# cmhungsteve/TA3N

Measured on NVIDIA H100. Metric: video-clips/sec fwd+bwd (B=256,T=5,D=2048), higher is better.
Workload: dtype tf32x3

## Files before the change

### include/ta3n_b200.h

```cpp
#ifndef TA3N_B200_H_
#define TA3N_B200_H_

#include <stddef.h>
#include <stdint.h>

#ifdef __cplusplus
extern "C" {
#endif

#define TA3N_ABI_VERSION 3

enum {
  TA3N_OK = 0,
  TA3N_ERR_INVALID = 1,
  TA3N_ERR_WORKSPACE = 2,
  TA3N_ERR_CUDA = 3,
  TA3N_ERR_UNSUPPORTED = 4
};

enum {
  TA3N_GEMM_FP32_SIMT = 0,
  TA3N_GEMM_TF32_TCGEN05 = 1,
  TA3N_GEMM_TF32X3_TCGEN05 = 2
};

typedef void* ta3n_stream_t;

typedef struct {
  int num_frames;
  int n_scales;
  const int* scale_size;
  const int* rel_count;
  const int* frames;
} ta3n_relation_table;

typedef struct {
  float p;
  const uint8_t* keep;
  uint64_t seed;
  const uint64_t* step_dev;
} ta3n_dropout;

int ta3n_abi_version(void);
const char* ta3n_last_error(void);
uint64_t ta3n_launch_count(void);
void ta3n_reset_launch_count(void);
int ta3n_set_gemm_engine(int engine);
int ta3n_get_gemm_engine(void);
int ta3n_set_forward_scratch(void* scratch, size_t bytes);
int ta3n_plan_forward_splits(int n_groups, const int* M, const int* N, const int* K, int sms, size_t scratch_bytes,
                             int* ksplit_out, double* makespan_out);
void ta3n_timing_enable(int on);
size_t ta3n_timing_report(char* buf, size_t buf_bytes);

int ta3n_shared_fc_fwd(const float* x_src, int rows_src, const float* x_tgt, int rows_tgt, int D,
                       const float* W, const float* b, int F, const ta3n_dropout* drop,
                       float* feat, ta3n_stream_t stream);
size_t ta3n_shared_fc_bwd_workspace_bytes(int rows, int D, int F);
int ta3n_shared_fc_bwd(const float* x_src, int rows_src, const float* x_tgt, int rows_tgt, int D,
                       int F, const float* feat, float* dfeat, const float* g_feat_ext, float p,
                       float* dW, float* db, void* workspace, size_t workspace_bytes,
                       ta3n_stream_t stream);

int ta3n_disc_fwd(const float* x, int rows, int K, int Kh, const float* W1, const float* b1,
                  const float* W2, const float* b2, float* hidden, float* logits,
                  ta3n_stream_t stream);
size_t ta3n_disc_bwd_workspace_bytes(int rows, int K, int Kh);
int ta3n_disc_bwd(const float* x, int rows, int K, int Kh, const float* W1, const float* W2,
                  const float* hidden, const float* g_logits, float beta, float* dx,
                  int accumulate, float* dW1, float* db1, float* dW2, float* db2,
                  void* workspace, size_t workspace_bytes, ta3n_stream_t stream);
int ta3n_grl_bwd(const float* g, float beta, float* out, size_t n, ta3n_stream_t stream);

int ta3n_frame_attn_fwd(const float* feat, const float* logits, int rows, int F, float* out,
                        ta3n_stream_t stream);
int ta3n_frame_attn_bwd(const float* feat, const float* logits, int rows, int F, float* d_out,
                        float* g_logits, ta3n_stream_t stream);

int ta3n_segment_mean_fwd(const float* x, int M, int T, int F, float* out, ta3n_stream_t stream);
int ta3n_segment_mean_bwd(const float* g, int M, int T, int F, float* dx, ta3n_stream_t stream);

int ta3n_trn_fwd(const float* x, int M, int F, int H, const ta3n_relation_table* tab,
                 const float* const* W_host, const float* const* b_host, int relu_input,
                 float* act, float* feat_rel, ta3n_stream_t stream);
size_t ta3n_trn_bwd_workspace_bytes(int M, int F, int H, const ta3n_relation_table* tab);
int ta3n_trn_bwd(const float* x, int M, int F, int H, const ta3n_relation_table* tab,
                 const float* const* W_host, int relu_input, const float* act,
                 const float* d_feat_rel, float* const* dW_host, float* const* db_host, float* dx,
                 int accumulate_dx, void* workspace, size_t workspace_bytes, ta3n_stream_t stream);

int ta3n_relattn_fwd(const float* feat_rel, int M, int R, int H, const float* const* W1_host,
                     const float* const* b1_host, const float* const* W2_host,
                     const float* const* b2_host, int use_attn, float* hidden, float* pred_rel,
                     float* attn, float* feat_video, ta3n_stream_t stream);
size_t ta3n_relattn_bwd_workspace_bytes(int M, int R, int H);
int ta3n_relattn_bwd(const float* feat_rel, int M, int R, int H, const float* const* W1_host,
                     const float* const* W2_host, int use_attn, const float* hidden,
                     const float* pred_rel, const float* attn, const float* g_feat_video,
                     const float* g_pred_rel, const float* g_attn, float beta,
                     float* d_feat_rel, float* const* dW1_host, float* const* db1_host,
                     float* const* dW2_host, float* const* db2_host, void* workspace,
                     size_t workspace_bytes, ta3n_stream_t stream);

int ta3n_general_attn_fwd(const float* feat_rel, int M, int R, int H, const float* W1, const float* b1,
                          const float* w2, const float* b2, float* hidden, float* attn, float* feat_video,
                          ta3n_stream_t stream);
size_t ta3n_general_attn_bwd_workspace_bytes(int M, int R, int H);
int ta3n_general_attn_bwd(const float* feat_rel, int M, int R, int H, const float* W1, const float* w2,
                          const float* hidden, const float* attn, const float* g_feat_video, const float* g_attn,
                          float* d_feat_rel, float* dW1, float* db1, float* dw2, float* db2, void* workspace,
                          size_t workspace_bytes, ta3n_stream_t stream);

int ta3n_video_head_fwd(const float* feat_video, int M, int H, int C, const float* Wc,
                        const float* bc, const ta3n_dropout* drop, float* dropped, float* pred,
                        ta3n_stream_t stream);
size_t ta3n_video_head_bwd_workspace_bytes(int M, int H, int C);
int ta3n_video_head_bwd(const float* dropped, int M, int H, int C, const float* Wc,
                        const ta3n_dropout* drop, const float* g_pred,
                        const float* d_dropped_extra, const float* g_feat_video_ext,
                        float grad_scale, float* d_feat_video, float* dWc, float* dbc,
                        void* workspace, size_t workspace_bytes, ta3n_stream_t stream);

int ta3n_fwd_batch_begin(void);
size_t ta3n_fwd_batch_workspace_bytes(void);
int ta3n_fwd_batch_flush(void* workspace, size_t workspace_bytes, ta3n_stream_t stream);

int ta3n_wgrad_defer_begin(void);
size_t ta3n_wgrad_defer_workspace_bytes(void);
int ta3n_wgrad_defer_flush(void* workspace, size_t workspace_bytes, ta3n_stream_t stream);

size_t ta3n_loss_workspace_bytes(int M);
int ta3n_loss_fwd_bwd(const float* pred_video, const long long* labels, const float* pred_rel,
                      const float* pred_dom_video, const float* pred_frame, int Bs, int Bt, int T,
                      int R, int C, float gamma, int flags, const int* valid_rows, float* loss,
                      float* g_pred_video,
                      float* g_pred_rel, float* g_pred_dom_video, float* g_pred_frame,
                      void* workspace, size_t workspace_bytes, ta3n_stream_t stream);
int ta3n_counter_inc(uint64_t* counter, ta3n_stream_t stream);

typedef struct {
  int Bs, Bt;
  int T, D, F, H, C;
  int use_attn;
  int loss_flags;
  float gamma;
  float domain_weight[2];
  const float* class_weight;
  const float* beta_dev;
  const ta3n_relation_table* tab;
  const float* x_src;
  const float* x_tgt;
  const long long* labels;
  const int* valid_rows;
  ta3n_dropout drop_i, drop_v;
  const float *W_sh, *b_sh;
  const float *W1f, *b1f, *W2f, *b2f;
  const float* const* W_trn_host;
  const float* const* b_trn_host;
  const float* const* W1r_host;
  const float* const* b1r_host;
  const float* const* W2r_host;
  const float* const* b2r_host;
  const float *Wc, *bc;
  const float *W1v, *b1v, *W2v, *b2v;
  float *dW_sh, *db_sh, *dW1f, *db1f, *dW2f, *db2f;
  float* const* dW_trn_host;
  float* const* db_trn_host;
  float* const* dW1r_host;
  float* const* db1r_host;
  float* const* dW2r_host;
  float* const* db2r_host;
  float *dWc, *dbc, *dW1v, *db1v, *dW2v, *db2v;
  float* feat;
  float* hid_f;
  float* pred_frame;
  float* act;
  float* feat_rel;
  float* hid_r;
  float* pred_rel;
  float* attn;
  float* feat_video;
  float* dropped;
  float* pred_video;
  float* hid_v;
  float* pred_dom;
  float* loss;
  uint64_t* step_counter;
  void* workspace;
  size_t workspace_bytes;
} ta3n_step_desc;

size_t ta3n_step_workspace_bytes(const ta3n_step_desc* desc);
int ta3n_step_run_phased(const ta3n_step_desc* desc, ta3n_stream_t stream);

size_t ta3n_allreduce_flag_bytes(int world);
int ta3n_allreduce_mean(float* const* peer_bufs_host, float* multicast_buf, uint32_t* const* peer_flags_host,
                        const uint64_t* seq_dev, int rank, int world, long long n, ta3n_stream_t stream);

size_t ta3n_sgd_workspace_bytes(void);
// ... 20 lines not shown
```

### ta3n_b200/_lib.py

```python
from __future__ import annotations

import ctypes as C
import os
import threading

from . import build as _build

ABI_VERSION = 3

TA3N_GEMM_FP32_SIMT = 0
TA3N_GEMM_TF32_TCGEN05 = 1
TA3N_GEMM_TF32X3_TCGEN05 = 2


class RelationTable(C.Structure):
    _fields_ = [("num_frames", C.c_int), ("n_scales", C.c_int),
                ("scale_size", C.POINTER(C.c_int)), ("rel_count", C.POINTER(C.c_int)),
                ("frames", C.POINTER(C.c_int))]


class Dropout(C.Structure):
    _fields_ = [("p", C.c_float), ("keep", C.c_void_p), ("seed", C.c_uint64), ("step_dev", C.c_void_p)]


class StepDesc(C.Structure):
    _fields_ = (
        [(n, C.c_int) for n in ("Bs", "Bt", "T", "D", "F", "H", "C", "use_attn", "loss_flags")] +
        [("gamma", C.c_float), ("domain_weight", C.c_float * 2), ("class_weight", C.c_void_p),
         ("beta_dev", C.c_void_p), ("tab", C.POINTER(RelationTable)),
         ("x_src", C.c_void_p), ("x_tgt", C.c_void_p), ("labels", C.c_void_p), ("valid_rows", C.c_void_p),
         ("drop_i", Dropout), ("drop_v", Dropout)] +
        [(n, C.c_void_p) for n in ("W_sh", "b_sh", "W1f", "b1f", "W2f", "b2f")] +
        [(n, C.POINTER(C.c_void_p)) for n in ("W_trn_host", "b_trn_host", "W1r_host", "b1r_host", "W2r_host",
                                              "b2r_host")] +
        [(n, C.c_void_p) for n in ("Wc", "bc", "W1v", "b1v", "W2v", "b2v")] +
        [(n, C.c_void_p) for n in ("dW_sh", "db_sh", "dW1f", "db1f", "dW2f", "db2f")] +
        [(n, C.POINTER(C.c_void_p)) for n in ("dW_trn_host", "db_trn_host", "dW1r_host", "db1r_host", "dW2r_host",
                                              "db2r_host")] +
        [(n, C.c_void_p) for n in ("dWc", "dbc", "dW1v", "db1v", "dW2v", "db2v")] +
        [(n, C.c_void_p) for n in ("feat", "hid_f", "pred_frame", "act", "feat_rel", "hid_r", "pred_rel", "attn",
                                   "feat_video", "dropped", "pred_video", "hid_v", "pred_dom", "loss",
                                   "step_counter", "workspace")] +
        [("workspace_bytes", C.c_size_t)])


_VP, _I, _F, _SZ = C.c_void_p, C.c_int, C.c_float, C.c_size_t
_IP = C.POINTER(C.c_int)
_PP = C.POINTER(C.c_void_p)
_TAB = C.POINTER(RelationTable)
_DRP = C.POINTER(Dropout)

SIGNATURES = {
    "ta3n_abi_version": (_I, []),
    "ta3n_last_error": (C.c_char_p, []),
    "ta3n_launch_count": (C.c_uint64, []),
    "ta3n_reset_launch_count": (None, []),
    "ta3n_set_gemm_engine": (_I, [_I]),
    "ta3n_get_gemm_engine": (_I, []),
    "ta3n_set_forward_scratch": (_I, [_VP, _SZ]),
    "ta3n_plan_forward_splits": (_I, [_I, _IP, _IP, _IP, _I, _SZ, _IP, C.POINTER(C.c_double)]),
    "ta3n_timing_enable": (None, [_I]),
    "ta3n_timing_report": (_SZ, [C.c_char_p, _SZ]),
    "ta3n_shared_fc_fwd": (_I, [_VP, _I, _VP, _I, _I, _VP, _VP, _I, _DRP, _VP, _VP]),
    "ta3n_shared_fc_bwd_workspace_bytes": (_SZ, [_I, _I, _I]),
    "ta3n_shared_fc_bwd": (_I, [_VP, _I, _VP, _I, _I, _I, _VP, _VP, _VP, _F, _VP, _VP, _VP, _SZ, _VP]),
    "ta3n_disc_fwd": (_I, [_VP, _I, _I, _I, _VP, _VP, _VP, _VP, _VP, _VP, _VP]),
    "ta3n_disc_bwd_workspace_bytes": (_SZ, [_I, _I, _I]),
    "ta3n_disc_bwd": (_I, [_VP, _I, _I, _I, _VP, _VP, _VP, _VP, _F, _VP, _I, _VP, _VP, _VP, _VP, _VP, _SZ, _VP]),
    "ta3n_grl_bwd": (_I, [_VP, _F, _VP, _SZ, _VP]),
    "ta3n_frame_attn_fwd": (_I, [_VP, _VP, _I, _I, _VP, _VP]),
    "ta3n_frame_attn_bwd": (_I, [_VP, _VP, _I, _I, _VP, _VP, _VP]),
    "ta3n_segment_mean_fwd": (_I, [_VP, _I, _I, _I, _VP, _VP]),
    "ta3n_segment_mean_bwd": (_I, [_VP, _I, _I, _I, _VP, _VP]),
    "ta3n_trn_fwd": (_I, [_VP, _I, _I, _I, _TAB, _PP, _PP, _I, _VP, _VP, _VP]),
    "ta3n_trn_bwd_workspace_bytes": (_SZ, [_I, _I, _I, _TAB]),
    "ta3n_trn_bwd": (_I, [_VP, _I, _I, _I, _TAB, _PP, _I, _VP, _VP, _PP, _PP, _VP, _I, _VP, _SZ, _VP]),
    "ta3n_relattn_fwd": (_I, [_VP, _I, _I, _I, _PP, _PP, _PP, _PP, _I, _VP, _VP, _VP, _VP, _VP]),
    "ta3n_relattn_bwd_workspace_bytes": (_SZ, [_I, _I, _I]),
    "ta3n_relattn_bwd": (_I, [_VP, _I, _I, _I, _PP, _PP, _I, _VP, _VP, _VP, _VP, _VP, _VP, _F, _VP,
                              _PP, _PP, _PP, _PP, _VP, _SZ, _VP]),
    "ta3n_general_attn_fwd": (_I, [_VP, _I, _I, _I, _VP, _VP, _VP, _VP, _VP, _VP, _VP, _VP]),
    "ta3n_general_attn_bwd_workspace_bytes": (_SZ, [_I, _I, _I]),
    "ta3n_general_attn_bwd": (_I, [_VP, _I, _I, _I, _VP, _VP, _VP, _VP, _VP, _VP, _VP, _VP, _VP, _VP, _VP, _VP, _SZ, _VP]),
    "ta3n_video_head_fwd": (_I, [_VP, _I, _I, _I, _VP, _VP, _DRP, _VP, _VP, _VP]),
    "ta3n_video_head_bwd_workspace_bytes": (_SZ, [_I, _I, _I]),
    "ta3n_video_head_bwd": (_I, [_VP, _I, _I, _I, _VP, _DRP, _VP, _VP, _VP, _F, _VP, _VP, _VP, _VP, _SZ, _VP]),
    "ta3n_fwd_batch_begin": (_I, []),
    "ta3n_fwd_batch_workspace_bytes": (_SZ, []),
    "ta3n_fwd_batch_flush": (_I, [_VP, _SZ, _VP]),
    "ta3n_wgrad_defer_begin": (_I, []),
    "ta3n_wgrad_defer_workspace_bytes": (_SZ, []),
    "ta3n_wgrad_defer_flush": (_I, [_VP, _SZ, _VP]),
    "ta3n_loss_workspace_bytes": (_SZ, [_I]),
    "ta3n_loss_fwd_bwd": (_I, [_VP, _VP, _VP, _VP, _VP, _I, _I, _I, _I, _I, _F, _I, _VP, _VP, _VP, _VP, _VP, _VP,
                               _VP, _SZ, _VP]),
    "ta3n_counter_inc": (_I, [_VP, _VP]),
    "ta3n_step_workspace_bytes": (_SZ, [C.POINTER(StepDesc)]),
    "ta3n_step_run_phased": (_I, [C.POINTER(StepDesc), _VP]),
    "ta3n_allreduce_flag_bytes": (_SZ, [_I]),
    "ta3n_allreduce_mean": (_I, [_PP, _VP, _PP, _VP, _I, _I, C.c_longlong, _VP]),
    "ta3n_sgd_workspace_bytes": (_SZ, []),
    "ta3n_sgd_nesterov_step": (_I, [_VP, _VP, _VP, C.c_longlong, _VP, _F, _F, _F, _VP, _SZ, _VP, _VP]),
    "ta3n_sgd_nesterov_step_masked": (_I, [_VP, _VP, _VP, C.c_longlong, _VP, _F, _F, _F, _VP, _SZ, _VP, _VP, _VP]),
    "ta3n_gemm_tn": (_I, [_VP, _VP, _VP, _I, _I, _I, _VP]),
    "ta3n_gemm_ex": (_I, [_VP, _I, _I, _VP, _I, _I, _VP, _I, _I, _I, _I, _VP, _SZ, _VP]),
}

_lock = threading.Lock()
_lib = None


class Ta3nError(RuntimeError):
    pass


def lib_path() -> str:
    return os.environ.get("TA3N_LIB", _build.LIB_PATH)


def load() -> C.CDLL:
    global _lib
    if _lib is not None:
        return _lib
    with _lock:
        if _lib is None:
            path = lib_path()
            if not os.path.exists(path):
                raise Ta3nError(
                    f"{path} is missing: build it with `python -m ta3n_b200.build` "
                    "(or __graft_entry__.build()). ta3n_b200 has no CPU / PyTorch fallback.")
            lib = C.CDLL(path)
            for name, (res, args) in SIGNATURES.items():
                fn = getattr(lib, name)
                fn.restype = res
                fn.argtypes = args
            if lib.ta3n_abi_version() != ABI_VERSION:
                raise Ta3nError("libta3n_sm90.so ABI version mismatch")
            _lib = lib
    return _lib


def check(rc: int) -> None:
    if rc != 0:
        msg = load().ta3n_last_error()
        raise Ta3nError(f"libta3n_sm90 error {rc}: {msg.decode() if msg else '?'}")


def ptr_array(ptrs):
    arr = (C.c_void_p * len(ptrs))(*ptrs)
    return arr


def set_gemm_engine(engine) -> None:
    code = {"fp32": TA3N_GEMM_FP32_SIMT, "tf32": TA3N_GEMM_TF32_TCGEN05, "tf32x3": TA3N_GEMM_TF32X3_TCGEN05}.get(engine, engine)
    check(load().ta3n_set_gemm_engine(int(code)))


def get_gemm_engine() -> str:
    return {0: "fp32", 1: "tf32", 2: "tf32x3"}[load().ta3n_get_gemm_engine()]


def plan_forward_splits(shapes, sms: int = 132, scratch_bytes: int = 48 << 20):
    n = len(shapes)
    arr = lambda col: (C.c_int * n)(*[int(s[col]) for s in shapes])
    ks, span = (C.c_int * n)(), (C.c_double * 2)()
    check(load().ta3n_plan_forward_splits(n, arr(0), arr(1), arr(2), int(sms), int(scratch_bytes), ks, span))
    return list(ks), span[0], span[1]

# ... 22 lines not shown
```

### ta3n_b200/build.py

```python
from __future__ import annotations

import os
import shutil
import subprocess
import sys

PKG_DIR = os.path.dirname(os.path.abspath(__file__))
CSRC = os.path.join(PKG_DIR, "csrc")
LIB_PATH = os.path.join(PKG_DIR, "libta3n_sm90.so")
SOURCES = ["ta3n_api.cu"]
HEADERS = ["common.cuh", "seg_gemm.cuh", "rowops.cuh", "gemm_wgmma.cuh", "optim.cuh", "step_rows.cuh",
           "step_plan.cuh", "allreduce.cuh",
           os.path.join("..", "..", "include", "ta3n_b200.h")]
NVCC_FLAGS = [
    "-gencode", "arch=compute_90a,code=sm_90a", "-lineinfo", "-O3", "-std=c++17",
    "-Xcompiler", "-fPIC", "-shared",
]


def _nvcc() -> str:
    for cand in (shutil.which("nvcc"), "/usr/local/cuda/bin/nvcc"):
        if cand and os.path.exists(cand):
            return cand
    raise RuntimeError("nvcc not found; cannot build libta3n_sm90.so")


def needs_build() -> bool:
    if not os.path.exists(LIB_PATH):
        return True
    t = os.path.getmtime(LIB_PATH)
    deps = [os.path.join(CSRC, s) for s in SOURCES + HEADERS]
    return any(os.path.getmtime(d) > t for d in deps if os.path.exists(d))


def build(force: bool = False, verbose: bool = False) -> str:
    if not force and not needs_build():
        return LIB_PATH
    cmd = [_nvcc(), *NVCC_FLAGS, *[os.path.join(CSRC, s) for s in SOURCES], "-o", LIB_PATH]
    if verbose:
        cmd.insert(1, "-Xptxas")
        cmd.insert(2, "-v")
        print(" ".join(cmd), file=sys.stderr)
    res = subprocess.run(cmd, capture_output=True, text=True)
    if res.returncode != 0:
        raise RuntimeError("nvcc failed:\n" + res.stdout + res.stderr)
    if verbose:
        print(res.stderr, file=sys.stderr)
    return LIB_PATH


if __name__ == "__main__":
    print(build(force="--force" in sys.argv, verbose=True))
```

### ta3n_b200/csrc/ta3n_api.cu

```cuda
#include "common.cuh"
#include "seg_gemm.cuh"
#include "rowops.cuh"
#include "gemm_wgmma.cuh"
#include "optim.cuh"
#include "step_plan.cuh"
#include "allreduce.cuh"

#include <functional>

using namespace ta3n;

namespace {

struct RelLayout {
  int T, R, n_rel, n_slots;
  std::vector<int> scale_size, rel_count, rel_begin;
  std::vector<int> rel_scale;
  std::vector<int> slot_begin;
  const int* frames;
};

int parse_table(const ta3n_relation_table* tab, RelLayout* L) {
  TA3N_REQUIRE(tab != nullptr, "relation table is null");
  TA3N_REQUIRE(tab->num_frames >= 2 && tab->n_scales >= 1 && tab->n_scales <= kMaxScales, "bad table sizes");
  TA3N_REQUIRE(tab->scale_size && tab->rel_count && tab->frames, "relation table arrays are null");
  L->T = tab->num_frames;
  L->R = tab->n_scales;
  L->frames = tab->frames;
  L->n_rel = 0;
  L->n_slots = 0;
  for (int i = 0; i < L->R; ++i) {
    const int s = tab->scale_size[i], n = tab->rel_count[i];
    TA3N_REQUIRE(s >= 1 && s <= L->T && n >= 1, "bad scale entry");
    L->scale_size.push_back(s);
    L->rel_count.push_back(n);
    L->rel_begin.push_back(L->n_rel);
    for (int r = 0; r < n; ++r) {
      L->rel_scale.push_back(i);
      L->slot_begin.push_back(L->n_slots);
      for (int j = 0; j < s; ++j) {
        const int t = tab->frames[L->n_slots + j];
        TA3N_REQUIRE(t >= 0 && t < L->T, "frame id out of range");
      }
      L->n_slots += s;
    }
    L->n_rel += n;
  }
  L->rel_begin.push_back(L->n_rel);
  TA3N_REQUIRE(L->n_rel <= kMaxRel, "too many relations");
  return TA3N_OK;
}

RelMap make_relmap(const RelLayout& L) {
  RelMap m;
  memset(&m, 0, sizeof(m));
  m.n_rel = L.n_rel;
  m.n_scales = L.R;
  for (int i = 0; i <= L.R; ++i) m.rel_begin[i] = L.rel_begin[i];
  for (int q = 0; q < L.n_rel; ++q) m.scale_of[q] = (unsigned char)L.rel_scale[q];
  return m;
}

void set_dropout_epilogue(Group& g, const DropArgs& d, const uint8_t* keep, int ldkeep, uint64_t rng_offset) {
  if (d.mode == 0) return;
  g.drop_scale = d.scale;
  g.drop_p = d.p;
  if (d.mode == 1) {
    g.flags |= EPI_DROP_MASK;
    g.keep = keep;
    g.ldkeep = ldkeep;
  } else {
    g.flags |= EPI_DROP_RNG;
    g.seed = d.seed;
    g.step_dev = d.step_dev;
    g.rng_offset = rng_offset;
  }
}

inline cudaStream_t S(ta3n_stream_t s) { return static_cast<cudaStream_t>(s); }

inline size_t splitk_bytes(int n_groups) {
  return (size_t)2 * 296 * 128 * 128 * sizeof(float) + (size_t)256 * (n_groups + 1) + 4096;
}

struct DeferCtx {
// ... 644 lines not shown
    plan.precise = true;
    Group& g = plan.add_group(M * R, H, hidden, H);
    g.flags = EPI_BIAS;
    g.bias = b1;
    plan.add_seg(feat_rel, H, W1, H, H);
    TA3N_TRY(run_gemm(plan, S(stream)));
  }
  pre_launch("general_attn_rows", S(stream));
  launch_kernel(general_attn_fwd_kernel, M, 32 * (R < kRelWarps ? R : kRelWarps), 0, S(stream), feat_rel, hidden, M, R,
                H, w2, b2, attn, feat_video);
  return after_launch();
}

size_t ta3n_general_attn_bwd_workspace_bytes(int M, int R, int H) {
  return Arena::round((size_t)M * R * H * sizeof(float)) + Arena::round((size_t)M * R * sizeof(float)) +
         splitk_bytes(1) + colsum_bytes((size_t)2 * H + 1);
}

int ta3n_general_attn_bwd(const float* feat_rel, int M, int R, int H, const float* W1, const float* w2,
                          const float* hidden, const float* attn, const float* g_feat_video, const float* g_attn,
                          float* d_feat_rel, float* dW1, float* db1, float* dw2, float* db2, void* workspace,
                          size_t workspace_bytes, ta3n_stream_t stream) {
  TA3N_REQUIRE(M >= 0 && R >= 1 && R <= kMaxScales && H > 0, "bad sizes");
  TA3N_REQUIRE(dW1 && db1 && dw2 && db2, "null gradient pointer");
  cudaStream_t st = S(stream);
  if (M == 0) {
    TA3N_CUDA(cudaMemsetAsync(dW1, 0, sizeof(float) * H * H, st));
    TA3N_CUDA(cudaMemsetAsync(db1, 0, sizeof(float) * H, st));
    TA3N_CUDA(cudaMemsetAsync(dw2, 0, sizeof(float) * H, st));
    TA3N_CUDA(cudaMemsetAsync(db2, 0, sizeof(float), st));
    return TA3N_OK;
  }
  TA3N_REQUIRE(feat_rel && W1 && w2 && hidden && attn && g_feat_video && d_feat_rel, "null pointer");
  Arena arena(workspace, workspace_bytes);
  float* d_pre = arena.floats((size_t)M * R * H);
  float* d_s = arena.floats((size_t)M * R);
  if (!d_pre || !d_s)
    return fail(TA3N_ERR_WORKSPACE, "ta3n_general_attn_bwd: workspace too small (%zu bytes)", workspace_bytes);
  pre_launch("general_attn_bwd_rows", st);
  launch_kernel(general_attn_bwd_kernel, M, 32 * (R < kRelWarps ? R : kRelWarps), 0, st, feat_rel, hidden, attn,
                g_feat_video, g_attn, M, R, H, w2, d_s, d_pre);
  TA3N_TRY(after_launch());
  {
    GemmPlan plan;
    plan.label = "general_attn_wgrad";
    plan.a_kmaj = false;
    plan.b_kmaj = false;
    plan.add_group(H, H, dW1, H);
    plan.add_seg(d_pre, H, feat_rel, H, M * R);
    TA3N_TRY(submit_wgrad(plan, st, &arena));
  }
  {
    ColsumPlan cs;
    cs.add_weighted(dw2, H, 1, H, H, 1);
    cs.seg(hidden, M * R, d_s);
    cs.add(db2, 1, 1);
    cs.seg(d_s, M * R);
    cs.add(db1, H, H);
    cs.seg(d_pre, M * R);
    TA3N_TRY(submit_colsum(cs, st, &arena));
  }
  {
    GemmPlan plan;
    plan.label = "general_attn_dgrad";
    plan.precise_dgrad = true;
    plan.a_kmaj = true;
    plan.b_kmaj = false;
    Group& g = plan.add_group(M * R, H, d_feat_rel, H);
    g.flags = EPI_ACCUM;
    plan.add_seg(d_pre, H, W1, H, H);
    TA3N_TRY(run_gemm(plan, st));
  }
  return TA3N_OK;
}

int ta3n_video_head_fwd(const float* feat_video, int M, int H, int C, const float* Wc, const float* bc,
                        const ta3n_dropout* drop, float* dropped, float* pred, ta3n_stream_t stream) {
  TA3N_REQUIRE(M >= 0 && H > 0 && C > 0, "bad sizes");
  if (M == 0) return TA3N_OK;
  TA3N_REQUIRE(feat_video && Wc && bc && dropped && pred, "null pointer");
  const DropArgs d = make_drop(drop);
  TA3N_REQUIRE(feat_video != dropped, "dropped must not alias feat_video");
  return launch_head_fwd(feat_video, H, Wc, bc, pred, C, M, H, C, S(stream), &d, dropped);
}

size_t ta3n_video_head_bwd_workspace_bytes(int M, int H, int C) {
  (void)M;
  return splitk_bytes(1) + colsum_bytes((size_t)C * (H + 1));
}

int ta3n_video_head_bwd(const float* dropped, int M, int H, int C, const float* Wc, const ta3n_dropout* drop,
                        const float* g_pred, const float* d_dropped_extra, const float* g_feat_video_ext,
                        float grad_scale, float* d_feat_video, float* dWc, float* dbc, void* workspace,
                        size_t workspace_bytes, ta3n_stream_t stream) {
  TA3N_REQUIRE(M >= 0 && H > 0 && C > 0, "bad sizes");
  TA3N_REQUIRE(dWc && dbc, "null gradient pointer");
  cudaStream_t st = S(stream);
  if (M == 0 || g_pred == nullptr) {
    TA3N_CUDA(cudaMemsetAsync(dWc, 0, sizeof(float) * C * H, st));
    TA3N_CUDA(cudaMemsetAsync(dbc, 0, sizeof(float) * C, st));
  }
  if (M == 0) return TA3N_OK;
  TA3N_REQUIRE(dropped && Wc && d_feat_video, "null pointer");
  const DropArgs d = make_drop(drop);
  pre_launch("video_head_bwd", st);
  launch_kernel(video_head_bwd_kernel, blocks_for((size_t)M * H, 256), 256, 0, st, g_pred, C, Wc, d_dropped_extra,
                                                                         g_feat_video_ext, grad_scale, d,
                                                                         d_feat_video, M, H);
  TA3N_TRY(after_launch());
  if (g_pred) {
    Arena arena(workspace, workspace_bytes);
    if (C <= 32) {
      ColsumPlan cs;
      cs.add_weighted(dWc, H, C, H, H, C);
      cs.seg(dropped, M, g_pred);
      cs.add(dbc, C, C);
      cs.seg(g_pred, M);
      TA3N_TRY(submit_colsum(cs, st, &arena));
    } else {
      GemmPlan plan;
      plan.label = "video_head_wgrad";
      plan.a_kmaj = false;
      plan.b_kmaj = false;
      plan.add_group(C, H, dWc, H);
      plan.add_seg(g_pred, C, dropped, H, M);
      TA3N_TRY(submit_wgrad(plan, st, &arena));
      ColsumPlan cs;
      cs.add(dbc, C, C);
      cs.seg(g_pred, M);
      TA3N_TRY(submit_colsum(cs, st, &arena));
    }
  }
  return TA3N_OK;
}

size_t ta3n_loss_workspace_bytes(int M) { return Arena::round((size_t)M * sizeof(float)) + 256; }

int ta3n_loss_fwd_bwd(const float* pred_video, const long long* labels, const float* pred_rel,
                      const float* pred_dom_video, const float* pred_frame, int Bs, int Bt, int T, int R, int C,
                      float gamma, int flags, const int* valid_rows, float* loss, float* g_pred_video,
                      float* g_pred_rel, float* g_pred_dom_video, float* g_pred_frame, void* workspace,
                      size_t workspace_bytes, ta3n_stream_t stream) {
  TA3N_REQUIRE(Bs >= 1 && Bt >= 0 && T >= 1 && R >= 1 && C >= 1, "bad sizes");
  TA3N_REQUIRE(pred_video && labels && pred_rel && pred_dom_video && pred_frame && loss, "null input");
  TA3N_REQUIRE(g_pred_video && g_pred_rel && g_pred_dom_video && g_pred_frame, "null gradient output");
  const int M = Bs + Bt;
  Arena arena(workspace, workspace_bytes);
  float* row_loss = arena.floats(M);
  if (!row_loss) return fail(TA3N_ERR_WORKSPACE, "ta3n_loss_fwd_bwd: workspace too small (%zu bytes)", workspace_bytes);
  pre_launch("loss_heads", S(stream));
  launch_kernel(loss_heads_kernel, blocks_for((size_t)M * 32, 256), 256, 0, S(stream), 
      pred_video, labels, pred_rel, pred_dom_video, pred_frame, Bs, M, T, R, C, gamma, flags, valid_rows,
      g_pred_video, g_pred_rel, g_pred_dom_video, g_pred_frame, row_loss);
  TA3N_TRY(after_launch());
  pre_launch("loss_reduce", S(stream));
  launch_kernel(loss_reduce_kernel, 1, 1024, 0, S(stream), row_loss, M, loss);
  return after_launch();
}

int ta3n_counter_inc(uint64_t* counter, ta3n_stream_t stream) {
  TA3N_REQUIRE(counter != nullptr, "null counter");
  pre_launch("counter_inc", S(stream));
  launch_kernel(counter_inc_kernel, 1, 1, 0, S(stream), reinterpret_cast<unsigned long long*>(counter));
  return after_launch();
}

// ... 160 lines not shown
```

### ta3n_b200/functional.py

```python
from __future__ import annotations

import ctypes as C
import itertools
import math
from dataclasses import dataclass, field
from functools import lru_cache
from typing import List, Optional, Sequence, Tuple

import torch

from . import _lib
from ._lib import Dropout, RelationTable, check, ptr_array


class RelationSet:

    def __init__(self, num_frames: int, subsample: int = 3):
        if num_frames < 2:
            raise ValueError("TRN needs at least 2 frames")
        self.num_frames = num_frames
        self.scales = list(range(num_frames, 1, -1))
        self.tuples: List[List[Tuple[int, ...]]] = []
        for pos, s in enumerate(self.scales):
            combos = list(itertools.combinations(range(num_frames), s))
# ... 131 lines not shown
    use_attn: bool = True
    general_attn: bool = False
    use_attn_frame: bool = False
    drop_i: DropSpec = field(default_factory=DropSpec)
    drop_v: DropSpec = field(default_factory=DropSpec)


def _attn_layer_params(params, R):
    n = 6 + 6 * R + 6
    if len(params) != n + 4:
        raise _lib.Ta3nError(f"general attention expects {n + 4} parameter tensors, got {len(params)}")
    return params[n:n + 4]


def _split_params(params, R):
    it = iter(params)
    take = lambda n: [next(it) for _ in range(n)]
    shared = take(2)
    fdisc = take(4)
    trn_w, trn_b = take(R), take(R)
    r_w1, r_b1, r_w2, r_b2 = take(R), take(R), take(R), take(R)
    cls = take(2)
    vdisc = take(4)
    return shared, fdisc, trn_w, trn_b, r_w1, r_b1, r_w2, r_b2, cls, vdisc


class Buffers:

    def __init__(self, device, persistent: bool = False):
        self.device = device
        self.persistent = persistent
        self.pool = {}

    def get(self, name, *shape, dtype=torch.float32):
        if not self.persistent:
            return torch.empty(*shape, device=self.device, dtype=dtype)
        t = self.pool.get(name)
        if t is None or tuple(t.shape) != tuple(shape) or t.dtype != dtype:
            t = torch.empty(*shape, device=self.device, dtype=dtype)
            self.pool[name] = t
        return t

    def workspace(self, name, nbytes):
        return self.get("ws_" + name, max(int(nbytes), 256), dtype=torch.uint8)


def path_forward(spec: PathSpec, xs, xt, params, bufs: Buffers, batch_gemms: bool = False):
    lib = _lib.load()
    st = _stream()
    T = spec.num_segments
    if xs.dim() != 3 or xt.dim() != 3 or xs.shape[1] != T or xt.shape[1] != T or xs.shape[2] != xt.shape[2]:
        raise _lib.Ta3nError(f"inputs must be (B,{T},D); got {tuple(xs.shape)} and {tuple(xt.shape)}")
    Bs, Bt, D = xs.shape[0], xt.shape[0], xs.shape[2]
    M, R = Bs + Bt, T - 1
    rs = relation_set(T)
    (w_sh, b_sh), (w1f, b1f, w2f, b2f), trn_w, trn_b, r_w1, r_b1, r_w2, r_b2, (w_c, b_c), \
        (w1v, b1v, w2v, b2v) = _split_params(params, R)
    F, H, Cn = w_sh.shape[0], trn_w[0].shape[0], w_c.shape[0]
    new = bufs.get
    d_i, d_v = spec.drop_i.cstruct(), spec.drop_v.cstruct()

    feat = new("feat", M * T, F)
    check(lib.ta3n_shared_fc_fwd(_p(xs), Bs * T, _p(xt), Bt * T, D, _p(w_sh), _p(b_sh), F, _dref(d_i),
                                 _p(feat), st))
    hid_f, pred_frame = new("hid_f", M * T, F), new("pred_frame", M * T, 2)
    batched = batch_gemms and not spec.use_attn_frame
    if batched:
        check(lib.ta3n_fwd_batch_begin())
    check(lib.ta3n_disc_fwd(_p(feat), M * T, F, F, _p(w1f), _p(b1f), _p(w2f), _p(b2f), _p(hid_f),
                            _p(pred_frame), st))
    if spec.use_attn_frame:
        feat_in = new("feat_in", M * T, F)
        check(lib.ta3n_frame_attn_fwd(_p(feat), _p(pred_frame), M * T, F, _p(feat_in), st))
    else:
        feat_in = feat
    act, feat_rel = new("act", rs.n_rel, M, H), new("feat_rel", M, R, H)
    check(lib.ta3n_trn_fwd(_p(feat_in), M, F, H, rs.ref, ptr_array([_p(w) for w in trn_w]),
                           ptr_array([_p(b) for b in trn_b]), 0, _p(act), _p(feat_rel), st))
    if batched:
        ws = bufs.workspace("fwd_batch", lib.ta3n_fwd_batch_workspace_bytes())
        check(lib.ta3n_fwd_batch_flush(_p(ws), ws.numel(), st))
    hid_r, pred_rel = new("hid_r", R, M, H), new("pred_rel", M, R, 2)
    attn, feat_video = new("attn", M, R), new("feat_video", M, H)
    check(lib.ta3n_relattn_fwd(_p(feat_rel), M, R, H, ptr_array([_p(w) for w in r_w1]),
                               ptr_array([_p(b) for b in r_b1]), ptr_array([_p(w) for w in r_w2]),
                               ptr_array([_p(b) for b in r_b2]), int(spec.use_attn and not spec.general_attn),
                               _p(hid_r), _p(pred_rel), _p(attn), _p(feat_video), st))
    hid_a = None
    if spec.general_attn:
        wa1, ba1, wa2, ba2 = _attn_layer_params(params, R)
        hid_a = new("hid_a", M * R, H)
        check(lib.ta3n_general_attn_fwd(_p(feat_rel), M, R, H, _p(wa1), _p(ba1), _p(wa2), _p(ba2), _p(hid_a), _p(attn),
                                        _p(feat_video), st))
    dropped, pred_video = new("dropped", M, H), new("pred_video", M, Cn)
    check(lib.ta3n_video_head_fwd(_p(feat_video), M, H, Cn, _p(w_c), _p(b_c), _dref(d_v), _p(dropped),
                                  _p(pred_video), st))
    hid_v, pred_dom_video = new("hid_v", M, H), new("pred_dom_video", M, 2)
    check(lib.ta3n_disc_fwd(_p(dropped), M, H, H, _p(w1v), _p(b1v), _p(w2v), _p(b2v), _p(hid_v),
                            _p(pred_dom_video), st))

    saved = dict(feat=feat, hid_f=hid_f, pred_frame=pred_frame, feat_in=feat_in, act=act, feat_rel=feat_rel,
                 hid_r=hid_r, pred_rel=pred_rel, attn=attn, dropped=dropped, hid_v=hid_v)
    if hid_a is not None:
        saved["hid_a"] = hid_a
    outputs = (feat.view(M, T, F), pred_frame.view(M, T, 2), attn, pred_rel, feat_video, pred_video,
               pred_dom_video, dropped)
    return saved, outputs, (Bs, Bt, D, T, F, H, Cn)


def path_backward(spec: PathSpec, dims, xs, xt, params, saved, gin, gout, bufs: Buffers, stage_done=None,
                  side_stream=None):
    stage_done = stage_done or (lambda name: None)
    frame_parallel = side_stream is not None and not spec.use_attn_frame
    lib = _lib.load()
    st = _stream()
    Bs, Bt, D, T, F, H, Cn = dims
    M, R = Bs + Bt, T - 1
    rs = relation_set(T)
    (w_sh, b_sh), (w1f, b1f, w2f, b2f), trn_w, trn_b, r_w1, r_b1, r_w2, r_b2, (w_c, b_c), \
        (w1v, b1v, w2v, b2v) = _split_params(params, R)
    (dw_sh, db_sh), (dw1f, db1f, dw2f, db2f), dtrn_w, dtrn_b, dr_w1, dr_b1, dr_w2, dr_b2, (dw_c, db_c), \
        (dw1v, db1v, dw2v, db2v) = _split_params(gout, R)
    g = lambda k: gin.get(k)
    new, wsp = bufs.get, bufs.workspace
    d_v = spec.drop_v.cstruct()
    feat, hid_f, pred_frame, feat_in = saved["feat"], saved["hid_f"], saved["pred_frame"], saved["feat_in"]
    act, feat_rel, hid_r, pred_rel = saved["act"], saved["feat_rel"], saved["hid_r"], saved["pred_rel"]
    attn, dropped, hid_v = saved["attn"], saved["dropped"], saved["hid_v"]
    d_feat = new("d_feat", M * T, F)
    g_pf = g("pred_frame")
    if g_pf is not None:
        g_pf = g_pf.reshape(M * T, 2)

    def frame_disc_bwd(stream_handle, accumulate):
        ws_f = wsp("disc_f", lib.ta3n_disc_bwd_workspace_bytes(M * T, F, F))
        check(lib.ta3n_disc_bwd(_p(feat), M * T, F, F, _p(w1f), _p(w2f), _p(hid_f), _p(g_pf),
                                float(spec.beta[2]), _p(d_feat), accumulate, _p(dw1f), _p(db1f), _p(dw2f), _p(db2f),
                                _p(ws_f), ws_f.numel(), stream_handle))

    frame_done = None
    if frame_parallel:
        main = torch.cuda.current_stream()
        fork = torch.cuda.Event()
        fork.record(main)
        side_stream.wait_event(fork)
        frame_disc_bwd(side_stream.cuda_stream, 0)
        frame_done = torch.cuda.Event()
        frame_done.record(side_stream)

    d_dropped = new("d_dropped", M, H)
    g_dropped = g("dropped")
    if g_dropped is not None:
        d_dropped.copy_(g_dropped.reshape(M, H))
    ws = wsp("disc_v", lib.ta3n_disc_bwd_workspace_bytes(M, H, H))
    check(lib.ta3n_disc_bwd(_p(dropped), M, H, H, _p(w1v), _p(w2v), _p(hid_v), _p(g("pred_dom_video")),
                            float(spec.beta[1]), _p(d_dropped), 1 if g_dropped is not None else 0, _p(dw1v), _p(db1v),
                            _p(dw2v), _p(db2v), _p(ws), ws.numel(), st))
    G = new("G", M, H)
    ws = wsp("vhead", lib.ta3n_video_head_bwd_workspace_bytes(M, H, Cn))
    check(lib.ta3n_video_head_bwd(_p(dropped), M, H, Cn, _p(w_c), _dref(d_v), _p(g("pred_video")), _p(d_dropped),
                                  _p(g("feat_video")), float(-spec.mu) if spec.reverse else 1.0, _p(G),
                                  _p(dw_c), _p(db_c), _p(ws), ws.numel(), st))
    stage_done("video")
    d_feat_rel = new("d_feat_rel", M, R, H)
    ws = wsp("relattn", lib.ta3n_relattn_bwd_workspace_bytes(M, R, H))
    check(lib.ta3n_relattn_bwd(_p(feat_rel), M, R, H, ptr_array([_p(w) for w in r_w1]),
                               ptr_array([_p(w) for w in r_w2]), 2 if spec.general_attn else int(spec.use_attn),
                               _p(hid_r), _p(pred_rel),
                               _p(attn), _p(G), _p(g("pred_rel")), _p(g("attn")), float(spec.beta[0]),
                               _p(d_feat_rel), ptr_array([_p(t) for t in dr_w1]),
                               ptr_array([_p(t) for t in dr_b1]), ptr_array([_p(t) for t in dr_w2]),
                               ptr_array([_p(t) for t in dr_b2]), _p(ws), ws.numel(), st))
    if spec.general_attn:
        wa1, _, wa2, _ = _attn_layer_params(params, R)
        dwa1, dba1, dwa2, dba2 = _attn_layer_params(gout, R)
        ws = wsp("general_attn", lib.ta3n_general_attn_bwd_workspace_bytes(M, R, H))
        check(lib.ta3n_general_attn_bwd(_p(feat_rel), M, R, H, _p(wa1), _p(wa2), _p(saved["hid_a"]), _p(attn), _p(G),
                                        _p(g("attn")), _p(d_feat_rel), _p(dwa1), _p(dba1), _p(dwa2), _p(dba2),
                                        _p(ws), ws.numel(), st))
    stage_done("relation")
    if frame_done is not None:
        torch.cuda.current_stream().wait_event(frame_done)
# ... 214 lines not shown
```

Before: 1.072 million.

## Fuse relation-attention, video head and video discriminator forward into one cluster kernel

```diff
diff --git a/include/ta3n_b200.h b/include/ta3n_b200.h
--- a/include/ta3n_b200.h
+++ b/include/ta3n_b200.h
@@ -8,7 +8,7 @@
 extern "C" {
 #endif
 
-#define TA3N_ABI_VERSION 3
+#define TA3N_ABI_VERSION 4
 
 enum {
   TA3N_OK = 0,
@@ -115,6 +115,13 @@
                         const float* bc, const ta3n_dropout* drop, float* dropped, float* pred,
                         ta3n_stream_t stream);
 size_t ta3n_video_head_bwd_workspace_bytes(int M, int H, int C);
+
+int ta3n_video_fwd(const float* feat_rel, int M, int R, int H, const float* const* W1r_host,
+                   const float* const* b1r_host, const float* const* W2r_host, const float* const* b2r_host, int C,
+                   const float* Wc, const float* bc, const float* W1v, const float* b1v, const float* W2v,
+                   const float* b2v, int use_attn, const ta3n_dropout* drop, float* hid_r, float* pred_rel,
+                   float* attn, float* feat_video, float* dropped, float* pred_video, float* hid_v,
+                   float* pred_dom_video, ta3n_stream_t stream);
 int ta3n_video_head_bwd(const float* dropped, int M, int H, int C, const float* Wc,
                         const ta3n_dropout* drop, const float* g_pred,
                         const float* d_dropped_extra, const float* g_feat_video_ext,
diff --git a/ta3n_b200/_lib.py b/ta3n_b200/_lib.py
--- a/ta3n_b200/_lib.py
+++ b/ta3n_b200/_lib.py
@@ -6,7 +6,7 @@
 
 from . import build as _build
 
-ABI_VERSION = 3
+ABI_VERSION = 4
 
 TA3N_GEMM_FP32_SIMT = 0
 TA3N_GEMM_TF32_TCGEN05 = 1
@@ -84,6 +84,8 @@
     "ta3n_general_attn_bwd": (_I, [_VP, _I, _I, _I, _VP, _VP, _VP, _VP, _VP, _VP, _VP, _VP, _VP, _VP, _VP, _VP, _SZ, _VP]),
     "ta3n_video_head_fwd": (_I, [_VP, _I, _I, _I, _VP, _VP, _DRP, _VP, _VP, _VP]),
     "ta3n_video_head_bwd_workspace_bytes": (_SZ, [_I, _I, _I]),
+    "ta3n_video_fwd": (_I, [_VP, _I, _I, _I, _PP, _PP, _PP, _PP, _I, _VP, _VP, _VP, _VP, _VP, _VP, _I, _DRP,
+                            _VP, _VP, _VP, _VP, _VP, _VP, _VP, _VP, _VP]),
     "ta3n_video_head_bwd": (_I, [_VP, _I, _I, _I, _VP, _DRP, _VP, _VP, _VP, _F, _VP, _VP, _VP, _VP, _SZ, _VP]),
     "ta3n_fwd_batch_begin": (_I, []),
     "ta3n_fwd_batch_workspace_bytes": (_SZ, []),
diff --git a/ta3n_b200/build.py b/ta3n_b200/build.py
--- a/ta3n_b200/build.py
+++ b/ta3n_b200/build.py
@@ -9,7 +9,7 @@
 CSRC = os.path.join(PKG_DIR, "csrc")
 LIB_PATH = os.path.join(PKG_DIR, "libta3n_sm90.so")
 SOURCES = ["ta3n_api.cu"]
-HEADERS = ["common.cuh", "seg_gemm.cuh", "rowops.cuh", "gemm_wgmma.cuh", "optim.cuh", "step_rows.cuh",
+HEADERS = ["common.cuh", "seg_gemm.cuh", "rowops.cuh", "video_fwd.cuh", "gemm_wgmma.cuh", "optim.cuh", "step_rows.cuh",
            "step_plan.cuh", "allreduce.cuh",
            os.path.join("..", "..", "include", "ta3n_b200.h")]
 NVCC_FLAGS = [
diff --git a/ta3n_b200/csrc/ta3n_api.cu b/ta3n_b200/csrc/ta3n_api.cu
--- a/ta3n_b200/csrc/ta3n_api.cu
+++ b/ta3n_b200/csrc/ta3n_api.cu
@@ -1,6 +1,7 @@
 #include "common.cuh"
 #include "seg_gemm.cuh"
 #include "rowops.cuh"
+#include "video_fwd.cuh"
 #include "gemm_wgmma.cuh"
 #include "optim.cuh"
 #include "step_plan.cuh"
@@ -811,6 +812,113 @@
   const DropArgs d = make_drop(drop);
   TA3N_REQUIRE(feat_video != dropped, "dropped must not alias feat_video");
   return launch_head_fwd(feat_video, H, Wc, bc, pred, C, M, H, C, S(stream), &d, dropped);
+}
+
+int ta3n_video_fwd(const float* feat_rel, int M, int R, int H, const float* const* W1r_host,
+                   const float* const* b1r_host, const float* const* W2r_host, const float* const* b2r_host, int C,
+                   const float* Wc, const float* bc, const float* W1v, const float* b1v, const float* W2v,
+                   const float* b2v, int use_attn, const ta3n_dropout* drop, float* hid_r, float* pred_rel,
+                   float* attn, float* feat_video, float* dropped, float* pred_video, float* hid_v,
+                   float* pred_dom_video, ta3n_stream_t stream) {
+  TA3N_REQUIRE(M >= 0 && R >= 1 && R <= kMaxScales && H > 0 && C > 0, "bad sizes");
+  TA3N_REQUIRE(use_attn == 0 || use_attn == 1, "use_attn must be 0 or 1");
+  if (H != 64 && H != 128 && H != 256)
+    return fail(TA3N_ERR_UNSUPPORTED, "ta3n_video_fwd: H = %d must be 64, 128 or 256", H);
+  const size_t smem = video_fwd_smem_bytes(H, C);
+  if (smem > kVfMaxSmemBytes)
+    return fail(TA3N_ERR_UNSUPPORTED, "ta3n_video_fwd: C = %d classes need %zu bytes of shared memory per CTA", C, smem);
+  if (M == 0) return TA3N_OK;
+  TA3N_REQUIRE(feat_rel && W1r_host && b1r_host && W2r_host && b2r_host && Wc && bc && W1v && b1v && W2v && b2v,
+               "null input");
+  TA3N_REQUIRE(hid_r && pred_rel && attn && feat_video && dropped && pred_video && hid_v && pred_dom_video,
+               "null output");
+  TA3N_REQUIRE(feat_video != dropped, "dropped must not alias feat_video");
+  const int CL = H / kVfNS;
+  VideoFwdArgs a;
+  memset(&a, 0, sizeof(a));
+  bool aligned = aligned16(feat_rel) && aligned16(W1v) && aligned16(b1v) && aligned16(W2v) && aligned16(hid_r) &&
+                 aligned16(hid_v) && aligned16(feat_video) && aligned16(dropped);
+  for (int i = 0; i < R; ++i) {
+    TA3N_REQUIRE(W1r_host[i] && b1r_host[i] && W2r_host[i] && b2r_host[i], "null weight pointer");
+    a.W1r[i] = W1r_host[i];
+    a.b1r[i] = b1r_host[i];
+    a.W2r[i] = W2r_host[i];
+    a.b2r[i] = b2r_host[i];
+    aligned = aligned && aligned16(W1r_host[i]) && aligned16(b1r_host[i]) && aligned16(W2r_host[i]);
+  }
+  if (!aligned) return fail(TA3N_ERR_UNSUPPORTED, "ta3n_video_fwd: tensors must be 16-byte aligned");
+  a.feat_rel = feat_rel;
+  a.Wc = Wc;
+  a.bc = bc;
+  a.W1v = W1v;
+  a.b1v = b1v;
+  a.W2v = W2v;
+  a.b2v = b2v;
+  a.hid_r = hid_r;
+  a.pred_rel = pred_rel;
+  a.attn = attn;
+  a.feat_video = feat_video;
+  a.dropped = dropped;
+  a.pred_video = pred_video;
+  a.hid_v = hid_v;
+  a.pred_dom = pred_dom_video;
+  a.M = M;
+  a.R = R;
+  a.H = H;
+  a.C = C;
+  a.use_attn = use_attn;
+  a.drop = make_drop(drop);
+  cudaLaunchConfig_t cfg;
+  memset(&cfg, 0, sizeof(cfg));
+  const int clusters = (M + kVfRows - 1) / kVfRows;
+  cfg.gridDim = dim3((unsigned)(CL * clusters));
+  cfg.blockDim = dim3(kVfThreads);
+  cfg.dynamicSmemBytes = smem;
+  cfg.stream = S(stream);
+  cudaLaunchAttribute attr[2];
+  attr[0].id = cudaLaunchAttributeClusterDimension;
+  attr[0].val.clusterDim.x = CL;
+  attr[0].val.clusterDim.y = 1;
+  attr[0].val.clusterDim.z = 1;
+  cfg.attrs = attr;
+  cfg.numAttrs = 1;
+  int device = 0;
+  TA3N_CUDA(cudaGetDevice(&device));
+  int max_clusters = -1;
+  {
+    static std::mutex mu;
+    static std::vector<std::pair<std::pair<int, size_t>, int>> cache;
+    std::lock_guard<std::mutex> g(mu);
+    bool attr_set = false;
+    for (auto& c : cache) {
+      if (c.first.first != device) continue;
+      attr_set = true;
+      if (c.first.second == smem) max_clusters = c.second;
+    }
+    if (max_clusters < 0) {
+      if (!attr_set)
+        TA3N_CUDA(cudaFuncSetAttribute(video_fwd_kernel, cudaFuncAttributeMaxDynamicSharedMemorySize,
+                                       (int)kVfMaxSmemBytes));
+      cudaLaunchConfig_t q = cfg;
+      q.stream = nullptr;
+      TA3N_CUDA(cudaOccupancyMaxActiveClusters(&max_clusters, video_fwd_kernel, &q));
+      cache.push_back({{device, smem}, max_clusters});
+    }
+  }
+  if (clusters > max_clusters || gemm_engine().load() == TA3N_GEMM_TF32_TCGEN05) {
+    TA3N_TRY(ta3n_relattn_fwd(feat_rel, M, R, H, W1r_host, b1r_host, W2r_host, b2r_host, use_attn, hid_r, pred_rel, attn,
+                              feat_video, stream));
+    TA3N_TRY(ta3n_video_head_fwd(feat_video, M, H, C, Wc, bc, drop, dropped, pred_video, stream));
+    return ta3n_disc_fwd(dropped, M, H, H, W1v, b1v, W2v, b2v, hid_v, pred_dom_video, stream);
+  }
+  if (pdl_enabled()) {
+    attr[1].id = cudaLaunchAttributeProgrammaticStreamSerialization;
+    attr[1].val.programmaticStreamSerializationAllowed = 1;
+    cfg.numAttrs = 2;
+  }
+  pre_launch("video_fwd", S(stream));
+  cudaLaunchKernelEx(&cfg, video_fwd_kernel, a);
+  return after_launch();
 }
 
 size_t ta3n_video_head_bwd_workspace_bytes(int M, int H, int C) {
diff --git a/ta3n_b200/csrc/video_fwd.cuh b/ta3n_b200/csrc/video_fwd.cuh
--- /dev/null
+++ b/ta3n_b200/csrc/video_fwd.cuh
@@ -0,0 +1,265 @@
+#pragma once
+
+#include <cooperative_groups.h>
+
+#include "common.cuh"
+#include "rowops.cuh"
+
+namespace ta3n {
+
+namespace cg = cooperative_groups;
+
+constexpr int kVfKSplit = 8;
+constexpr int kVfThreads = 288;
+constexpr int kVfJN = 2;
+constexpr int kVfNS = 32 * kVfJN;
+constexpr int kVfRows = 18;
+static_assert(kVfRows * kVfNS == 4 * kVfThreads, "one float4 of hidden outputs per thread");
+
+struct VideoFwdArgs {
+  const float* feat_rel;
+  const float* W1r[kMaxScales];
+  const float* b1r[kMaxScales];
+  const float* W2r[kMaxScales];
+  const float* b2r[kMaxScales];
+  const float *Wc, *bc, *W1v, *b1v, *W2v, *b2v;
+  float *hid_r, *pred_rel, *attn, *feat_video, *dropped, *pred_video, *hid_v, *pred_dom;
+  int M, R, H, C, use_attn;
+  DropArgs drop;
+};
+
+inline size_t video_fwd_smem_bytes(int H, int C) {
+  return sizeof(float) * ((size_t)2 * kVfNS * (H + 4) + (size_t)2 * kVfRows * H + (size_t)kVfKSplit * kVfRows * kVfNS +
+                          4 * kVfRows + (size_t)C * (kVfNS + kVfRows));
+}
+constexpr int kVfMaxCluster = 4;
+constexpr size_t kVfMaxSmemBytes = 220 * 1024;
+
+__device__ __forceinline__ void vf_cp_async16(float* dst, const float* src, bool valid) {
+  const unsigned d = (unsigned)__cvta_generic_to_shared(dst);
+  const int n = valid ? 16 : 0;
+  asm volatile("cp.async.cg.shared.global [%0], [%1], 16, %2;" ::"r"(d), "l"(src), "r"(n) : "memory");
+}
+__device__ __forceinline__ void vf_cp_commit() { asm volatile("cp.async.commit_group;" ::: "memory"); }
+template <int N>
+__device__ __forceinline__ void vf_cp_wait() { asm volatile("cp.async.wait_group %0;" ::"n"(N) : "memory"); }
+
+__global__ void __launch_bounds__(kVfThreads, 1) video_fwd_kernel(const __grid_constant__ VideoFwdArgs a) {
+  extern __shared__ __align__(16) float vf_smem[];
+  __shared__ const float* tab[4][kMaxScales + 1];
+  cg::cluster_group cluster = cg::this_cluster();
+  const int H = a.H, R = a.R, M = a.M, C = a.C, ldw = H + 4;
+  const int CL = (int)cluster.num_blocks();
+  const int rank = (int)cluster.block_rank();
+  const int m0 = (blockIdx.x / CL) * kVfRows;
+  const int n0 = rank * kVfNS;
+  float* Wb = vf_smem;
+  float* Xb = Wb + 2 * kVfNS * ldw;
+  float* red = Xb + 2 * kVfRows * H;
+  float* lg = red + kVfKSplit * kVfRows * kVfNS;
+  float* wcs = lg + 4 * kVfRows;
+  float* cls = wcs + C * kVfNS;
+  const int tid = threadIdx.x, lane = tid & 31, warp = tid >> 5;
+  const int eq = tid % (kVfNS / 4), em = tid / (kVfNS / 4);
+  const bool erow = m0 + em < M;
+  const int q4 = H / 4, lrs = 256 / q4, lr0 = tid < 256 ? tid / q4 : kVfRows + kVfNS, lk4 = tid % q4;
+
+  for (int t = tid; t < 4 * (R + 1); t += kVfThreads) {
+    const int st = t >> 2, kind = t & 3;
+    const float* p;
+    if (st < R) p = kind == 0 ? a.W1r[st] : kind == 1 ? a.b1r[st] : kind == 2 ? a.W2r[st] : a.b2r[st];
+    else p = kind == 0 ? a.W1v : kind == 1 ? a.b1v : kind == 2 ? a.W2v : a.b2v;
+    tab[kind][st] = p;
+  }
+  __syncthreads();
+
+  auto load_w = [&](int buf, const float* W) {
+    float* dst = Wb + buf * kVfNS * ldw;
+    for (int n = lr0; n < kVfNS; n += lrs) vf_cp_async16(dst + n * ldw + 4 * lk4, W + (size_t)(n0 + n) * H + 4 * lk4, true);
+  };
+  auto load_x = [&](int buf, int i) {
+    float* dst = Xb + buf * kVfRows * H;
+    for (int m = lr0; m < kVfRows; m += lrs) {
+      const bool ok = m0 + m < M;
+      vf_cp_async16(dst + m * H + 4 * lk4, ok ? a.feat_rel + ((size_t)(m0 + m) * R + i) * H + 4 * lk4 : a.feat_rel, ok);
+    }
+  };
+
+  pdl_wait();
+  load_w(0, tab[0][0]);
+  load_x(0, 0);
+  vf_cp_commit();
+
+  float4 fv = make_float4(0.f, 0.f, 0.f, 0.f);
+  const int h0 = n0 + 4 * eq;
+  for (int s = 0; s <= R; ++s) {
+    const int buf = s & 1;
+    __syncthreads();
+    if (s < R) {
+      load_w(buf ^ 1, tab[0][s + 1]);
+      if (s + 1 < R) {
+        load_x(buf ^ 1, s + 1);
+      } else {
+        for (int t = tid; t < C * (kVfNS / 4); t += kVfThreads) {
+          const int c = t / (kVfNS / 4), k4 = t % (kVfNS / 4);
+          vf_cp_async16(wcs + c * kVfNS + 4 * k4, a.Wc + (size_t)c * H + n0 + 4 * k4, true);
+        }
+      }
+      vf_cp_commit();
+      vf_cp_wait<1>();
+    } else {
+      vf_cp_wait<0>();
+    }
+    const float4 bv = __ldg(reinterpret_cast<const float4*>(tab[1][s] + h0));
+    const float c0 = __ldg(tab[3][s]), c1 = __ldg(tab[3][s] + 1);
+    __syncthreads();
+    const float* Ws = Wb + buf * kVfNS * ldw;
+    const float* Xs = Xb + buf * kVfRows * H;
+
+    if (warp < kVfKSplit) {
+      const int kw = H / kVfKSplit;
+      float acc[kVfRows][kVfJN];
+#pragma unroll
+      for (int m = 0; m < kVfRows; ++m)
+#pragma unroll
+        for (int j = 0; j < kVfJN; ++j) acc[m][j] = 0.f;
+      const float* xk = Xs + warp * kw;
+      const float* wk = Ws + lane * ldw + warp * kw;
+      for (int k = 0; k < kw; k += 4) {
+        float4 w[kVfJN];
+#pragma unroll
+        for (int j = 0; j < kVfJN; ++j) w[j] = *reinterpret_cast<const float4*>(wk + 32 * j * ldw + k);
+#pragma unroll
+        for (int m = 0; m < kVfRows; ++m) {
+          const float4 x = *reinterpret_cast<const float4*>(xk + m * H + k);
+#pragma unroll
+          for (int j = 0; j < kVfJN; ++j) {
+            acc[m][j] = fmaf(x.x, w[j].x, acc[m][j]);
+            acc[m][j] = fmaf(x.y, w[j].y, acc[m][j]);
+            acc[m][j] = fmaf(x.z, w[j].z, acc[m][j]);
+            acc[m][j] = fmaf(x.w, w[j].w, acc[m][j]);
+          }
+          if (m % 6 == 5) asm volatile("" ::: "memory");
+        }
+      }
+#pragma unroll
+      for (int m = 0; m < kVfRows; ++m)
+#pragma unroll
+        for (int j = 0; j < kVfJN; ++j) red[(warp * kVfRows + m) * kVfNS + lane + 32 * j] = acc[m][j];
+    }
+    const float4 u0 = __ldg(reinterpret_cast<const float4*>(tab[2][s] + h0));
+    const float4 u1 = __ldg(reinterpret_cast<const float4*>(tab[2][s] + H + h0));
+    __syncthreads();
+
+    float4 hv = *reinterpret_cast<const float4*>(red + em * kVfNS + 4 * eq);
+#pragma unroll
+    for (int w = 1; w < kVfKSplit; ++w) {
+      const float4 t = *reinterpret_cast<const float4*>(red + (w * kVfRows + em) * kVfNS + 4 * eq);
+      hv.x += t.x;
+      hv.y += t.y;
+      hv.z += t.z;
+      hv.w += t.w;
+    }
+    hv.x = fmaxf(hv.x + bv.x, 0.f);
+    hv.y = fmaxf(hv.y + bv.y, 0.f);
+    hv.z = fmaxf(hv.z + bv.z, 0.f);
+    hv.w = fmaxf(hv.w + bv.w, 0.f);
+    float* hid = s < R ? a.hid_r + (size_t)s * M * H : a.hid_v;
+    if (erow) *reinterpret_cast<float4*>(hid + (size_t)(m0 + em) * H + h0) = hv;
+    float p0 = hv.x * u0.x, p1 = hv.x * u1.x;
+    p0 = fmaf(hv.y, u0.y, p0);
+    p1 = fmaf(hv.y, u1.y, p1);
+    p0 = fmaf(hv.z, u0.z, p0);
+    p1 = fmaf(hv.z, u1.z, p1);
+    p0 = fmaf(hv.w, u0.w, p0);
+    p1 = fmaf(hv.w, u1.w, p1);
+#pragma unroll
+    for (int o = kVfNS / 8; o > 0; o >>= 1) {
+      p0 += __shfl_xor_sync(0xffffffffu, p0, o);
+      p1 += __shfl_xor_sync(0xffffffffu, p1, o);
+    }
+    float* lgs = lg + buf * 2 * kVfRows;
+    if (eq == 0) {
+      lgs[2 * em] = p0;
+      lgs[2 * em + 1] = p1;
+    }
+    cluster.sync();
+    float l0 = 0.f, l1 = 0.f;
+#pragma unroll
+    for (int r = 0; r < kVfMaxCluster; ++r) {
+      if (r < CL) {
+        const float* rl = cluster.map_shared_rank(lgs, r);
+        l0 += rl[2 * em];
+        l1 += rl[2 * em + 1];
+      }
+    }
+    l0 += c0;
+    l1 += c1;
+    const bool writer = erow && rank == 0 && eq == 0;
+
+    if (s == R) {
+      if (writer) {
+        a.pred_dom[(size_t)(m0 + em) * 2] = l0;
+        a.pred_dom[(size_t)(m0 + em) * 2 + 1] = l1;
+      }
+      break;
+    }
+    const float w = a.use_attn ? attn_from_logits(l0, l1).w : 0.f;
+    if (writer) {
+      const size_t o = (size_t)(m0 + em) * R + s;
+      a.pred_rel[o * 2] = l0;
+      a.pred_rel[o * 2 + 1] = l1;
+      a.attn[o] = a.use_attn ? w : Xs[em * H];
+    }
+    const float4 x = *reinterpret_cast<const float4*>(Xs + em * H + h0);
+    fv.x = fmaf(w + 1.0f, x.x, fv.x);
+    fv.y = fmaf(w + 1.0f, x.y, fv.y);
+    fv.z = fmaf(w + 1.0f, x.z, fv.z);
+    fv.w = fmaf(w + 1.0f, x.w, fv.w);
+
+    if (s == R - 1) {
+      const size_t e = (size_t)(m0 + em) * H + h0;
+      const float4 d = make_float4(fv.x * drop_factor(a.drop, e), fv.y * drop_factor(a.drop, e + 1),
+                                   fv.z * drop_factor(a.drop, e + 2), fv.w * drop_factor(a.drop, e + 3));
+      if (erow) {
+        *reinterpret_cast<float4*>(a.feat_video + e) = fv;
+        *reinterpret_cast<float4*>(a.dropped + e) = d;
+      }
+      float* plane = Xb + (buf ^ 1) * kVfRows * H;
+      *reinterpret_cast<float4*>(plane + em * H + h0) = d;
+      vf_cp_wait<0>();
+      __syncthreads();
+      for (int c = 0; c < C; ++c) {
+        const float4 u = *reinterpret_cast<const float4*>(wcs + c * kVfNS + 4 * eq);
+        float t = d.x * u.x;
+        t = fmaf(d.y, u.y, t);
+        t = fmaf(d.z, u.z, t);
+        t = fmaf(d.w, u.w, t);
+#pragma unroll
+        for (int o = kVfNS / 8; o > 0; o >>= 1) t += __shfl_xor_sync(0xffffffffu, t, o);
+        if (eq == 0) cls[em * C + c] = t;
+      }
+      cluster.sync();
+#pragma unroll
+      for (int r = 0; r < kVfMaxCluster; ++r) {
+        if (r < CL && r != rank) {
+          const float* src = cluster.map_shared_rank(plane, r);
+          const int hr = r * kVfNS + 4 * eq;
+          *reinterpret_cast<float4*>(plane + em * H + hr) = *reinterpret_cast<const float4*>(src + em * H + hr);
+        }
+      }
+      if (rank == 0 && erow) {
+        for (int c = eq; c < C; c += kVfNS / 4) {
+          float t = 0.f;
+#pragma unroll
+          for (int r = 0; r < kVfMaxCluster; ++r)
+            if (r < CL) t += cluster.map_shared_rank(cls, r)[em * C + c];
+          a.pred_video[(size_t)(m0 + em) * C + c] = t + __ldg(a.bc + c);
+        }
+      }
+    }
+  }
+  cluster.sync();
+}
+
+}
diff --git a/ta3n_b200/functional.py b/ta3n_b200/functional.py
--- a/ta3n_b200/functional.py
+++ b/ta3n_b200/functional.py
@@ -237,22 +237,26 @@
         check(lib.ta3n_fwd_batch_flush(_p(ws), ws.numel(), st))
     hid_r, pred_rel = new("hid_r", R, M, H), new("pred_rel", M, R, 2)
     attn, feat_video = new("attn", M, R), new("feat_video", M, H)
-    check(lib.ta3n_relattn_fwd(_p(feat_rel), M, R, H, ptr_array([_p(w) for w in r_w1]),
-                               ptr_array([_p(b) for b in r_b1]), ptr_array([_p(w) for w in r_w2]),
-                               ptr_array([_p(b) for b in r_b2]), int(spec.use_attn and not spec.general_attn),
-                               _p(hid_r), _p(pred_rel), _p(attn), _p(feat_video), st))
+    dropped, pred_video = new("dropped", M, H), new("pred_video", M, Cn)
+    hid_v, pred_dom_video = new("hid_v", M, H), new("pred_dom_video", M, 2)
     hid_a = None
-    if spec.general_attn:
+    rel_tables = (ptr_array([_p(w) for w in r_w1]), ptr_array([_p(b) for b in r_b1]),
+                  ptr_array([_p(w) for w in r_w2]), ptr_array([_p(b) for b in r_b2]))
+    if not spec.general_attn:
+        check(lib.ta3n_video_fwd(_p(feat_rel), M, R, H, *rel_tables, Cn, _p(w_c), _p(b_c), _p(w1v), _p(b1v), _p(w2v),
+                                 _p(b2v), int(spec.use_attn), _dref(d_v), _p(hid_r), _p(pred_rel), _p(attn),
+                                 _p(feat_video), _p(dropped), _p(pred_video), _p(hid_v), _p(pred_dom_video), st))
+    else:
+        check(lib.ta3n_relattn_fwd(_p(feat_rel), M, R, H, *rel_tables, 0, _p(hid_r), _p(pred_rel), _p(attn),
+                                   _p(feat_video), st))
         wa1, ba1, wa2, ba2 = _attn_layer_params(params, R)
         hid_a = new("hid_a", M * R, H)
         check(lib.ta3n_general_attn_fwd(_p(feat_rel), M, R, H, _p(wa1), _p(ba1), _p(wa2), _p(ba2), _p(hid_a), _p(attn),
                                         _p(feat_video), st))
-    dropped, pred_video = new("dropped", M, H), new("pred_video", M, Cn)
-    check(lib.ta3n_video_head_fwd(_p(feat_video), M, H, Cn, _p(w_c), _p(b_c), _dref(d_v), _p(dropped),
-                                  _p(pred_video), st))
-    hid_v, pred_dom_video = new("hid_v", M, H), new("pred_dom_video", M, 2)
-    check(lib.ta3n_disc_fwd(_p(dropped), M, H, H, _p(w1v), _p(b1v), _p(w2v), _p(b2v), _p(hid_v),
-                            _p(pred_dom_video), st))
+        check(lib.ta3n_video_head_fwd(_p(feat_video), M, H, Cn, _p(w_c), _p(b_c), _dref(d_v), _p(dropped),
+                                      _p(pred_video), st))
+        check(lib.ta3n_disc_fwd(_p(dropped), M, H, H, _p(w1v), _p(b1v), _p(w2v), _p(b2v), _p(hid_v),
+                                _p(pred_dom_video), st))
 
     saved = dict(feat=feat, hid_f=hid_f, pred_frame=pred_frame, feat_in=feat_in, act=act, feat_rel=feat_rel,
                  hid_r=hid_r, pred_rel=pred_rel, attn=attn, dropped=dropped, hid_v=hid_v)
```

After: 1.120 million (median of 6 runs). +4.5%, better.
